# HongwenZhang/DaNet-DensePose2SMPL

Measured on AMD Instinct MI355X. Metric: images/sec fwd+bwd HRNet-W48+SMPL+IUV 256x256 bs32/GPU, higher is better.
Workload: dtype bf16; 1 GPU; full DaNet train step (HRNet-W48 + global and part-wise IUV heads + regressor nets + SMPL LBS (2 forward + 1 backward; the 2 label-side forwards belong to the untimed batch prologue) + IUV render + losses, fwd+bwd+Adam), 256x256, 32 img/GPU; convs bf16 MFMA fp32-acc, LBS/raster/losses fp32; global_batch=32, parallelism=dp1

## Files before the change

danet-densepose2smpl_amd/_lib.py:

```python
import ctypes
import os

_HERE = os.path.dirname(os.path.abspath(__file__))
LIB_PATH = os.environ.get('DANET_LIB') or os.path.join(_HERE, 'csrc', 'libdanet_hip.so')
_lib = None

c_f = ctypes.c_void_p
c_i = ctypes.c_int
c_sz = ctypes.c_size_t
c_fl = ctypes.c_float

_SIGNATURES = {
    'danet_version': (c_i, []),
    'danet_last_error': (ctypes.c_char_p, []),
    'danet_smpl_lbs_debug': (c_i, [c_f]),
    'danet_smpl_lbs_ctx_floats': (c_sz, [c_i]),
    'danet_smpl_lbs_fwd_ws_floats': (c_sz, [c_i, c_i, c_i]),
    'danet_smpl_lbs_bwd_ws_floats': (c_sz, [c_i, c_i, c_i]),
    'danet_smpl_lbs_ticket_words': (c_sz, [c_i]),
    'danet_smpl_lbs_forward': (c_i, [c_f, c_f, c_i] + [c_f] * 9 + [c_i] * 4 + [c_f] * 5 + [c_sz, c_f, c_f]),
    'danet_smpl_lbs_backward': (c_i, [c_f, c_f, c_i] + [c_f] * 7 + [c_i] * 4 + [c_f] * 7 + [c_sz, c_f, c_i, c_f]),
    'danet_smpl_lbs_backward_fused_ok': (c_i, [c_i, c_i, c_i]),
    'danet_iuv_raster_ws_bytes': (c_sz, [c_i, c_i, c_i]),
    'danet_iuv_raster_forward': (c_i, [c_f, c_f, c_i, c_i, c_f, c_i, c_f, c_f, c_i, c_fl, c_fl, c_i, c_f, c_f, c_f, c_f, c_sz, c_f]),
# ... 18 lines not shown
    'danet_conv_stem_ok': (c_i, [c_i] * 13),
    'danet_conv_stem_forward': (c_i, [c_f, c_f, c_f] + [c_i] * 7 + [c_f, c_f]),
    'danet_conv_stem_dgrad_ok': (c_i, [c_i] * 13),
    'danet_conv_stem_dgrad': (c_i, [c_f, c_f, c_f] + [c_i] * 7 + [c_f] * 5),
    'danet_conv3x3a_ok': (c_i, [c_i] * 11),
    'danet_conv3x3a': (c_i, [c_f, c_f, c_f] + [c_i] * 4 + [c_f] * 5 + [c_i, c_f, c_f]),
    'danet_conv3x3_stream_table_bytes': (c_sz, []),
    'danet_conv3x3_stream_tables': (c_i, [c_f, c_sz]),
    'danet_conv_pack_weights_batched': (c_i, [c_f, c_i, ctypes.c_long, ctypes.c_long, c_f]),
    'danet_conv_pack_job_bricks': (ctypes.c_long, [c_i] * 7),
    'danet_conv_forward_multi_ok': (c_i, [c_f, c_i]),
    'danet_conv_forward_multi_kernel': (c_i, [c_f, c_i]),
    'danet_conv_forward_multi': (c_i, [c_f, c_i, c_f]),
    'danet_conv_forward_multi_epi_ok': (c_i, [c_f, c_i]),
    'danet_conv_forward_multi_epi_kernel': (c_i, [c_f, c_i]),
    'danet_conv_forward_multi_epi': (c_i, [c_f, c_i, c_f]),
    'danet_conv_stem_forward_epi': (c_i, [c_f, c_f, c_f, c_f] + [c_i] * 8 + [c_f]),
    'danet_conv3x3a_forward_epi': (c_i, [c_f] * 5 + [c_i] * 4 + [c_f]),
    'danet_conv_bn_forward_multi_ok': (c_i, [c_f, c_i, c_f, c_f]),
    'danet_conv_bn_forward_multi': (c_i, [c_f, c_i, c_f, c_fl, c_fl, c_f, c_f, c_f]),
    'danet_conv_forward_kernel': (c_i, [c_i] * 15),
    'danet_conv_forward': (c_i, [c_f] * 4 + [c_i] * 16 + [c_f] * 6 + [c_i, c_f]),
    'danet_conv_wgrad_rows_ok': (c_i, [c_i] * 13),
    'danet_conv_wgrad_rows_ws_floats': (c_sz, [c_i] * 8),
    'danet_conv_wgrad_rows': (c_i, [c_f] * 4 + [c_sz] + [c_i] * 12 + [c_fl, c_f]),
    'danet_conv_wgrad3x3_ok': (c_i, [c_i] * 10),
    'danet_conv_wgrad3x3_pair_ok': (c_i, [c_i] * 11),
    'danet_conv_wgrad3x3_ws_floats': (c_sz, [c_i] * 7),
    'danet_conv_wgrad_multi_ws_floats': (c_sz, [c_f, c_i]),
    'danet_conv_wgrad_multi_ws_zero_from': (c_sz, [c_f, c_i]),
    'danet_conv_wgrad_multi': (c_i, [c_f, c_i, c_f, c_sz, c_fl, c_f]),
    'danet_conv_wgrad3x3_multi_ws_floats': (c_sz, [c_f, c_i]),
    'danet_conv_wgrad3x3_multi': (c_i, [c_f, c_i, c_f, c_sz, c_fl, c_f]),
    'danet_conv_wgrad3x3_kernel_id': (c_i, [c_i] * 7),
    'danet_conv_wgrad3x3': (c_i, [c_f] * 4 + [c_sz] + [c_i] * 7 + [c_fl, c_i, c_f]),
    'danet_conv_wgrad_ws_floats': (c_sz, [c_i] * 4),
    'danet_conv_wgrad_ws_floats_for': (c_sz, [c_i] * 13),
    'danet_conv_wgrad': (c_i, [c_f] * 4 + [c_sz] + [c_i] * 13 + [c_fl, c_i, c_f]),
    'danet_bn_forward': (c_i, [c_f, c_f, c_f, ctypes.c_int64, c_i] + [c_f] * 6 + [c_i, c_fl, c_fl, c_i, c_i, c_f, c_f]),
    'danet_bn_ws_floats': (c_sz, [c_i]),
    'danet_knob': (ctypes.c_long, [c_i, ctypes.c_long]),
    'danet_bn_acc_bytes': (c_i, []),
    'danet_channel_sum': (c_i, [c_f, ctypes.c_int64, c_i, c_f, c_i, c_i, c_f]),
    'danet_bn_forward_multi': (c_i, [c_f, c_i, c_fl, c_fl, c_f]),
    'danet_bn_backward_multi': (c_i, [c_f, c_i, c_f]),
    'danet_bn_backward_onepass_ok': (c_i, [c_f, c_i, c_i]),
    'danet_bn_backward_onepass_bar_words': (c_i, []),
    'danet_bn_backward_onepass': (c_i, [c_f, c_i, c_f, c_i, c_f]),
    'danet_bn_backward': (c_i, [c_f, c_f, c_f, ctypes.c_int64, c_i, c_f, c_f, c_i, c_f, c_f, c_f, c_f, c_i, c_i, c_f, c_f, c_f]),
    'danet_sum_relu_forward': (c_i, [ctypes.POINTER(ctypes.c_void_p), ctypes.POINTER(c_i), c_i, c_i, c_i, c_i, c_i, c_i, c_f, c_f]),
    'danet_sum_relu_backward': (c_i, [c_f, c_f, c_i, c_i, c_i, c_i, c_i, c_i, c_f, c_f]),
    'danet_sum_relu_backward_all': (c_i, [c_f, c_f] + [c_i] * 5 + [c_f] * 5),
    'danet_sum_relu_forward_multi': (c_i, [c_f, c_i, c_f]),
    'danet_sum_relu_backward_all_multi': (c_i, [c_f, c_i, c_f]),
    'danet_maxpool3x3s2_forward': (c_i, [c_f, c_f, c_f, c_i, c_i, c_i, c_i, c_f]),
    'danet_maxpool3x3s2_backward': (c_i, [c_f, c_f, c_f, c_i, c_i, c_i, c_i, c_f]),
    'danet_stn_gather_forward': (c_i, [c_f, c_f] + [c_i] * 8 + [c_f, c_f]),
    'danet_stn_gather_backward': (c_i, [c_f, c_f] + [c_i] * 8 + [c_f, c_f]),
    'danet_part_clean_forward': (c_i, [c_f, c_f, c_i, c_i, c_i, c_i, c_f, c_f]),
    'danet_part_clean_backward': (c_i, [c_f, c_f, c_f, c_i, c_i, c_i, c_i, c_f, c_f]),
    'danet_part_loss_forward': (c_i, [c_f] * 5 + [c_i] * 5 + [c_f, c_f]),
    'danet_part_loss_backward': (c_i, [c_f] * 6 + [c_i] * 5 + [c_f, c_f]),
    'danet_part_backward_fused': (c_i, [c_f] * 8 + [c_i] * 5 + [c_f, c_f]),
    'danet_part_gt_forward': (c_i, [c_f] * 5 + [c_i] * 4 + [c_f, c_f, c_f]),
    'danet_part_gt_backward': (c_i, [c_f] * 5 + [c_i] * 4 + [c_f, c_f]),
    'danet_iuv_global_forward': (c_i, [c_f] * 4 + [c_i, c_i] + [c_f] * 3 + [c_i] * 4 + [c_f] * 5),
# ... 301 lines not shown
```

danet-densepose2smpl_amd/csrc/conv_wgrad3x3.hip:

```cpp
#include <cstdlib>
#include "common.h"
#include "conv_common.h"

namespace {

using namespace danet_conv;

constexpr int TH = 4, TW = 8;
constexpr int halo_h(int st) { return st * (TH - 1) + 3; }
constexpr int halo_w(int st) { return st * (TW - 1) + 3; }

struct Wg3P {
    const bf16_t* x; const bf16_t* dy; float* part;
    float* direct;
    int B, H, W, Cin, Cout, groups, Cin_g, Cout_g;
    int IH, IW;
    int tiles_h, tiles_w, msplit;
    long nchunks;
    long x_bytes, dy_bytes;
};

typedef __attribute__((ext_vector_type(2))) unsigned v2u;

__device__ inline v2u tr_read(unsigned lds_byte_addr) {
    v2u r;
    asm volatile("ds_read_b64_tr_b16 %0, %1" : "=v"(r) : "v"(lds_byte_addr) : "memory");
    return r;
}

template <int CT, int NI, int ST, int SM = 0>
__device__ __forceinline__ void wgrad3x3_body(const Wg3P& p, const int bx, const int by, const int bz)
{
    constexpr bool PAIR = SM != 0;
// ... 143 lines not shown
            if (pair >= NPAIR || cin >= p.Cin_g) continue;
#pragma unroll
            for (int ct = 0; ct < CT; ++ct)
#pragma unroll
                for (int r = 0; r < 4; ++r) {
                    const int cout = co0 + ct * 16 + lg * 4 + r;
                    if (cout < p.Cout_g) dw[((size_t)cout * p.Cin_g + cin) * 9 + tap] = acc[pi][ct][r];
                }
        }
        return;
    }
    float* dst = p.part + ((size_t)bx * p.groups + g) * gsz;
#pragma unroll
    for (int pi = 0; pi < MAXP; ++pi) {
        const int pair = wave + 4 * pi;
        const int tap = pair / NI, ni = pair - tap * NI;
        const int cin = ci0 + ni * 16 + li;
        if (pair >= NPAIR || cin >= p.Cin_g) continue;
        float* row = dst + ((tap * p.Cout_g + co0 + lg * 4) * p.Cin_g + cin);
#pragma unroll
        for (int ct = 0; ct < CT; ++ct)
#pragma unroll
            for (int r = 0; r < 4; ++r)
                if (co0 + ct * 16 + lg * 4 + r < p.Cout_g) row[(ct * 16 + r) * p.Cin_g] = acc[pi][ct][r];
    }
}

template <int CT, int NI, int ST>
__global__ __launch_bounds__(256) void conv_wgrad3x3_kernel(Wg3P p)
{
    wgrad3x3_body<CT, NI, ST>(p, blockIdx.x, blockIdx.y, blockIdx.z);
}

constexpr int NPM = 20;
struct Wg3Multi { Wg3P p[NPM]; int start[NPM + 1]; int nyb[NPM]; int n; int xcd; };

template <int CT, int NI, int ST, int SM = 0>
__global__ __launch_bounds__(256) void conv_wgrad3x3_multi_kernel(Wg3Multi mp)
{
    int vb = (int)blockIdx.x;
    if (mp.xcd) {
        const int G = (int)gridDim.x, q = G >> 3, r = G & 7;
        const int x = vb & 7, slot = vb >> 3;
        vb = x * q + (x < r ? x : r) + slot;
    }
    int i = 0;
    while (i + 1 < mp.n && vb >= mp.start[i + 1]) ++i;
    const int l = vb - mp.start[i];
    const Wg3P& p = mp.p[i];
    const int bx = l % p.msplit, rest = l / p.msplit;
    wgrad3x3_body<CT, NI, ST, SM>(p, bx, rest % mp.nyb[i], rest / mp.nyb[i]);
}

struct Red3Multi { const float* part[NPM]; float* dw[NPM]; int G[NPM], Cout_g[NPM], Cin_g[NPM], msplit[NPM]; long start[NPM + 1]; int n; float beta; };

__global__ __launch_bounds__(256) void wgrad3x3_reduce_multi_kernel(Red3Multi rp)
{
    const long gidx = (long)blockIdx.x * 256 + threadIdx.x;
    if (gidx >= rp.start[rp.n]) return;
    int i = 0;
    while (i + 1 < rp.n && gidx >= rp.start[i + 1]) ++i;
    const long idx = gidx - rp.start[i], total = rp.start[i + 1] - rp.start[i];
    const float* part = rp.part[i];
    float s = 0.f;
    int sp = 0;
    for (; sp + 4 <= rp.msplit[i]; sp += 4) {
        const float v0 = part[(size_t)sp * total + idx], v1 = part[(size_t)(sp + 1) * total + idx];
        const float v2 = part[(size_t)(sp + 2) * total + idx], v3 = part[(size_t)(sp + 3) * total + idx];
        s += (v0 + v1) + (v2 + v3);
    }
    for (; sp < rp.msplit[i]; ++sp) s += part[(size_t)sp * total + idx];
    const int Cin_g = rp.Cin_g[i], Cout_g = rp.Cout_g[i];
    const int cin = (int)(idx % Cin_g);
    long rest = idx / Cin_g;
    const int cout = (int)(rest % Cout_g); rest /= Cout_g;
    const int tap = (int)(rest % 9), g = (int)(rest / 9);
    const size_t o = (((size_t)(g * Cout_g + cout)) * Cin_g + cin) * 9 + tap;
    float* dw = rp.dw[i];
    dw[o] = rp.beta != 0.f ? dw[o] * rp.beta + s : s;
}

__global__ __launch_bounds__(256) void wgrad3x3_reduce_kernel(const float* __restrict__ part, float* __restrict__ dw,
                                                               int G, int Cout_g, int Cin_g, int msplit, float beta)
{
    const long total = (long)G * Cout_g * Cin_g * 9;
    const long idx = (long)blockIdx.x * 256 + threadIdx.x;
    if (idx >= total) return;
    float s = 0.f;
    int sp = 0;
    for (; sp + 4 <= msplit; sp += 4) {
        const float v0 = part[(size_t)sp * total + idx], v1 = part[(size_t)(sp + 1) * total + idx];
        const float v2 = part[(size_t)(sp + 2) * total + idx], v3 = part[(size_t)(sp + 3) * total + idx];
        s += (v0 + v1) + (v2 + v3);
    }
    for (; sp < msplit; ++sp) s += part[(size_t)sp * total + idx];
    const int cin = (int)(idx % Cin_g);
    long rest = idx / Cin_g;
    const int cout = (int)(rest % Cout_g); rest /= Cout_g;
    const int tap = (int)(rest % 9), g = (int)(rest / 9);
    const size_t o = (((size_t)(g * Cout_g + cout)) * Cin_g + cin) * 9 + tap;
    dw[o] = beta != 0.f ? dw[o] * beta + s : s;
}

template <int CT, int NI, int ST>
int launch3(const Wg3P& p, hipStream_t st) {
    const int nco = (p.Cout_g + CT * 16 - 1) / (CT * 16), nci = (p.Cin_g + NI * 16 - 1) / (NI * 16);
    const size_t lds = 2 * (size_t)(TH * TW * CT * 32 + halo_h(ST) * halo_w(ST) * NI * 32);
    hipLaunchKernelGGL((conv_wgrad3x3_kernel<CT, NI, ST>), dim3(p.msplit, nco * nci, p.groups), dim3(256), lds, st, p);
    return 0;
}

inline int tiles3(int c) { return c <= 16 ? 1 : (c <= 32 ? 2 : ((c % 48 == 0 || c <= 48) ? 3 : 4)); }
// ... 60 lines not shown
    DANET_CHECK_ARG(danet_conv_wgrad3x3_ok(H, W, Cin, Cout, 3, 3, stride, 1, 1, groups), "conv_wgrad3x3: unsupported shape");
    Wg3P p;
    p.x = (const bf16_t*)x; p.dy = (const bf16_t*)dy; p.part = ws; p.direct = nullptr;
    p.IH = H; p.IW = W; H /= stride; W /= stride;
    p.B = B; p.H = H; p.W = W; p.Cin = Cin; p.Cout = Cout; p.groups = groups;
    p.Cin_g = Cin / groups; p.Cout_g = Cout / groups;
    p.tiles_h = H / TH; p.tiles_w = W / TW;
    p.nchunks = (long)B * p.tiles_h * p.tiles_w;
    p.x_bytes = (long)B * p.IH * p.IW * Cin * 2; p.dy_bytes = (long)B * H * W * Cout * 2;
    DANET_CHECK_ARG(p.x_bytes < (1L << 31) && p.dy_bytes < (1L << 31), "conv_wgrad3x3: tensors of 2 GB or more are not supported");
    int ct, ni;
    plan3(B, H, W, Cin, Cout, groups, &ct, &ni, &p.msplit);
    if (ws_floats < (size_t)p.msplit * Cout * p.Cin_g * 9)
        return danet::fail(DANET_ERR_WORKSPACE, "conv_wgrad3x3: workspace too small");
    hipStream_t st = (hipStream_t)stream;
    if (phase != 2) {
#define W3(a, b) if (ct == a && ni == b) { if (stride == 1) launch3<a, b, 1>(p, st); else launch3<a, b, 2>(p, st); } else
        W3(1, 1) W3(1, 2) W3(1, 3) W3(2, 1) W3(2, 2) W3(2, 3) W3(3, 1) W3(3, 2) W3(3, 3)
        return danet::fail(DANET_ERR_ARG, "conv_wgrad3x3: no kernel for tiles %dx%d", ct, ni);
#undef W3
        DANET_CHECK_LAUNCH("conv_wgrad3x3_kernel");
    }
    if (phase == 1) return DANET_OK;
    const long total = (long)Cout * p.Cin_g * 9;
    hipLaunchKernelGGL(wgrad3x3_reduce_kernel, dim3(danet::cdiv(total, 256)), dim3(256), 0, st, ws, dw, groups, p.Cout_g,
                       p.Cin_g, p.msplit, beta);
    DANET_CHECK_LAUNCH("wgrad3x3_reduce_kernel");
    return DANET_OK;
}


struct Wg3Job { const void* x; const void* dy; float* dw; int B, H, W, Cin, Cout, groups, stride; };

static long multi_target_blocks() {
    if (const char* e = getenv("DANET_WGRAD3_MULTI_BLOCKS")) return atol(e);
    return 768;
}

static inline double wg3_weight(int Cout, int Cin_g) { const double p = (double)Cout * Cin_g; return p < 2304.0 ? 2304.0 : p; }
static void plan_multi(const Wg3Job* jobs, const int* idx, int cnt, int ct, int ni, int* msplit) {
    auto chunks_of = [](const Wg3Job& j) -> long {
        const int sm = wg3_small(j.B, j.H, j.W, j.stride);
        return sm ? (long)(j.B / (sm == 4 ? 2 : 8)) : (long)j.B * (j.H / j.stride / TH) * (j.W / j.stride / TW);
    };
    double tot = 0;
    for (int k = 0; k < cnt; ++k) {
        const Wg3Job& j = jobs[idx[k]];
        tot += (double)chunks_of(j) * wg3_weight(j.Cout, j.Cin / j.groups);
    }
    const long target = multi_target_blocks();
    for (int k = 0; k < cnt; ++k) {
        const Wg3Job& j = jobs[idx[k]];
        const int Cout_g = j.Cout / j.groups, Cin_g = j.Cin / j.groups;
        const long other = (long)((Cout_g + ct * 16 - 1) / (ct * 16)) * ((Cin_g + ni * 16 - 1) / (ni * 16)) * j.groups;
        const long nchunks = chunks_of(j);
        const double w = (double)nchunks * wg3_weight(j.Cout, Cin_g);
        long ms = (long)(target * (w / tot) / other + 0.5);
        if (ms > nchunks / 4) ms = nchunks / 4;
        if (ms < 1) ms = 1;
        msplit[k] = (int)ms;
    }
}

static int multi_foreach_launch(const Wg3Job* jobs, int n, float* ws, size_t ws_floats, float beta, hipStream_t st, size_t* need_out)
{
    size_t used = 0;
    bool done[4096];
    if (n > 4096) return danet::fail(DANET_ERR_ARG, "conv_wgrad3x3_multi: too many jobs (%d)", n);
    for (int i = 0; i < n; ++i) done[i] = false;
    for (int i = 0; i < n; ++i) {
        if (done[i]) continue;
        int ct, ni, dummy;
        const int stride = jobs[i].stride;
        const int sm = wg3_small(jobs[i].B, jobs[i].H, jobs[i].W, stride);
        const bool pair = sm != 0;
        plan3(jobs[i].B, jobs[i].H / stride, jobs[i].W / stride, jobs[i].Cin, jobs[i].Cout, jobs[i].groups, &ct, &ni, &dummy);
        static const int npm_env = getenv("DANET_WGRAD3_NPM") ? atoi(getenv("DANET_WGRAD3_NPM")) : 0;
        const int npm = npm_env > 0 && npm_env < NPM ? npm_env : NPM;
        int idx[NPM], cnt = 0;
        for (int k = i; k < n && cnt < npm; ++k) {
            if (done[k] || jobs[k].stride != stride || wg3_small(jobs[k].B, jobs[k].H, jobs[k].W, stride) != sm) continue;
            int c2, n2;
            plan3(jobs[k].B, jobs[k].H / stride, jobs[k].W / stride, jobs[k].Cin, jobs[k].Cout, jobs[k].groups, &c2, &n2, &dummy);
            if (c2 == ct && n2 == ni) { idx[cnt++] = k; done[k] = true; }
        }
        int msplit[NPM];
        plan_multi(jobs, idx, cnt, ct, ni, msplit);
        Wg3Multi mp; Red3Multi rp;
        static const bool xcd_order = getenv("DANET_WGRAD3_XCD") && atoi(getenv("DANET_WGRAD3_XCD")) != 0;
        mp.n = cnt; rp.n = cnt; rp.beta = beta; mp.xcd = xcd_order ? 1 : 0;
        mp.start[0] = 0; rp.start[0] = 0;
        for (int k = 0; k < cnt; ++k) {
            const Wg3Job& j = jobs[idx[k]];
            Wg3P& p = mp.p[k];
            static const bool no_direct = getenv("DANET_WGRAD3_NO_DIRECT") != nullptr;
            const bool direct = msplit[k] == 1 && beta == 0.f && !no_direct;
            p.x = (const bf16_t*)j.x; p.dy = (const bf16_t*)j.dy; p.part = (ws && !direct) ? ws + used : nullptr;
            p.direct = direct ? j.dw : nullptr;
            p.IH = j.H; p.IW = j.W;
            p.B = j.B; p.H = j.H / stride; p.W = j.W / stride; p.Cin = j.Cin; p.Cout = j.Cout; p.groups = j.groups;
            if (pair) { p.B = j.B / (sm == 4 ? 2 : 8); p.H = 4; p.W = 8; p.IH = 4 * stride; p.IW = 8 * stride; }
            p.Cin_g = j.Cin / j.groups; p.Cout_g = j.Cout / j.groups;
            p.tiles_h = p.H / TH; p.tiles_w = p.W / TW;
            p.nchunks = (long)p.B * p.tiles_h * p.tiles_w;
            p.x_bytes = (long)j.B * j.H * j.W * j.Cin * 2; p.dy_bytes = (long)j.B * (j.H / stride) * (j.W / stride) * j.Cout * 2;
            p.msplit = msplit[k];
            const int nyb = ((p.Cout_g + ct * 16 - 1) / (ct * 16)) * ((p.Cin_g + ni * 16 - 1) / (ni * 16));
            mp.nyb[k] = nyb;
            mp.start[k + 1] = mp.start[k] + msplit[k] * nyb * j.groups;
            const long total = (long)j.Cout * p.Cin_g * 9;
            rp.part[k] = p.part; rp.dw[k] = j.dw; rp.G[k] = j.groups; rp.Cout_g[k] = p.Cout_g; rp.Cin_g[k] = p.Cin_g; rp.msplit[k] = msplit[k];
            rp.start[k + 1] = rp.start[k] + (direct ? 0 : total);
            if (!direct || !ws) used += (size_t)msplit[k] * total;
            if (ws && !(p.x_bytes < (1L << 31) && p.dy_bytes < (1L << 31)))
                return danet::fail(DANET_ERR_ARG, "conv_wgrad3x3_multi: tensors of 2 GB or more are not supported");
        }
        if (!ws) continue;
        if (used > ws_floats) return danet::fail(DANET_ERR_WORKSPACE, "conv_wgrad3x3_multi: workspace too small");
        const int phw = stride * ((sm ? sm : 4) - 1) + 3;
        const size_t lds = 2 * (size_t)(TH * TW * ct * 32 + (sm ? (TH / sm) * phw * (TW / sm) * phw : halo_h(stride) * halo_w(stride)) * ni * 32);
        const dim3 grid((unsigned)mp.start[cnt]);
        if (pair) {
#define W3P(a, b) if (ct == a && ni == b) { \
            if (stride == 1 && sm == 4) hipLaunchKernelGGL((conv_wgrad3x3_multi_kernel<a, b, 1, 4>), grid, dim3(256), lds, st, mp); \
            else if (stride == 2 && sm == 4) hipLaunchKernelGGL((conv_wgrad3x3_multi_kernel<a, b, 2, 4>), grid, dim3(256), lds, st, mp); \
            else if (stride == 1) hipLaunchKernelGGL((conv_wgrad3x3_multi_kernel<a, b, 1, 2>), grid, dim3(256), lds, st, mp); \
            else hipLaunchKernelGGL((conv_wgrad3x3_multi_kernel<a, b, 2, 2>), grid, dim3(256), lds, st, mp); } else
            W3P(2, 2) W3P(2, 3) W3P(3, 2) W3P(3, 3) W3P(1, 1) W3P(1, 2) W3P(2, 1) W3P(1, 3) W3P(3, 1)
            return danet::fail(DANET_ERR_ARG, "conv_wgrad3x3_multi: no pair-mode kernel for tiles %dx%d", ct, ni);
#undef W3P
        } else
#define W3M(a, b) if (ct == a && ni == b) { \
            if (stride == 1) hipLaunchKernelGGL((conv_wgrad3x3_multi_kernel<a, b, 1>), grid, dim3(256), lds, st, mp); \
            else hipLaunchKernelGGL((conv_wgrad3x3_multi_kernel<a, b, 2>), grid, dim3(256), lds, st, mp); } else
        W3M(1, 1) W3M(1, 2) W3M(1, 3) W3M(2, 1) W3M(2, 2) W3M(2, 3) W3M(3, 1) W3M(3, 2) W3M(3, 3)
        return danet::fail(DANET_ERR_ARG, "conv_wgrad3x3_multi: no kernel for tiles %dx%d", ct, ni);
#undef W3M
        DANET_CHECK_LAUNCH("conv_wgrad3x3_multi_kernel");
        if (rp.start[cnt] > 0) {
            hipLaunchKernelGGL(wgrad3x3_reduce_multi_kernel, dim3((unsigned)danet::cdiv(rp.start[cnt], 256)), dim3(256), 0, st, rp);
            DANET_CHECK_LAUNCH("wgrad3x3_reduce_multi_kernel");
        }
    }
    if (need_out) *need_out = used;
    return DANET_OK;
}

extern "C" size_t danet_conv_wgrad3x3_multi_ws_floats(const void* jobs, int n)
{
    size_t need = 0;
    if (!jobs || n <= 0) return 0;
    multi_foreach_launch((const Wg3Job*)jobs, n, nullptr, 0, 0.f, nullptr, &need);
    return need;
}

extern "C" int danet_conv_wgrad3x3_multi(const void* jobs, int n, float* ws, size_t ws_floats, float beta, void* stream)
{
    DANET_ENTER();
    DANET_CHECK_ARG(jobs && n > 0 && ws, "conv_wgrad3x3_multi: bad arguments");
    const Wg3Job* jb = (const Wg3Job*)jobs;
    for (int i = 0; i < n; ++i)
        DANET_CHECK_ARG(jb[i].x && jb[i].dy && jb[i].dw && jb[i].B > 0 &&
                        (danet_conv_wgrad3x3_ok(jb[i].H, jb[i].W, jb[i].Cin, jb[i].Cout, 3, 3, jb[i].stride, 1, 1, jb[i].groups) ||
                         danet_conv_wgrad3x3_pair_ok(jb[i].B, jb[i].H, jb[i].W, jb[i].Cin, jb[i].Cout, 3, 3, jb[i].stride, 1, 1, jb[i].groups)),
                        "conv_wgrad3x3_multi: job %d is not a supported 3x3 problem", i);
    return multi_foreach_launch(jb, n, ws, ws_floats, beta, (hipStream_t)stream, nullptr);
}
```

include/danet_hip.h:

```cpp
#ifndef DANET_HIP_H
#define DANET_HIP_H

#include <stddef.h>
#include <stdint.h>

#ifdef __cplusplus
extern "C" {
#endif

#define DANET_OK 0
#define DANET_ERR_ARG (-1)
#define DANET_ERR_HIP (-2)
#define DANET_ERR_WORKSPACE (-3)

int danet_version(void);
const char* danet_last_error(void);

size_t danet_smpl_lbs_ctx_floats(int B);
size_t danet_smpl_lbs_fwd_ws_floats(int B, int V, int NE);
size_t danet_smpl_lbs_bwd_ws_floats(int B, int V, int NB);
size_t danet_smpl_lbs_ticket_words(int B);

int danet_smpl_lbs_forward(const float* betas, const float* rotmats, int B,
                           const float* v_template, const float* shapedirs, const float* posedirs,
// ... 171 lines not shown
       DANET_KNOB_BN_BLOCK_BYTES = 15, DANET_KNOB_C3S_BALANCE = 16, DANET_KNOB_C3S_TILE_COST = 17,
       DANET_KNOB_G3 = 18  };
long danet_knob(int id, long value);
int danet_conv3x3_stream_plan(int B, int H, int W, int Cin, int Cout, int nprob);
size_t danet_conv3x3_stream_table_bytes(void);
int danet_conv3x3_stream_tables(void* workspace, size_t bytes);
int danet_conv_stem_ok(int B, int H, int W, int Cin, int OH, int OW, int Cout, int R, int S, int stride, int pad, int dil, int groups);
int danet_conv_stem_forward(const void* x, const void* wp, void* y, int B, int H, int W, int Cin, int OH, int OW, int Cout,
                            float* bn_sums, void* stream);
int danet_conv_stem_forward_epi(const void* x, const void* wp, const float* bias, void* y, int B, int H, int W, int Cin, int OH, int OW,
                                int Cout, int relu, void* stream);
int danet_conv_stem_dgrad_ok(int B, int H, int W, int Cin, int OH, int OW, int Cout, int R, int S, int stride, int pad, int dil, int groups);
int danet_conv_stem_dgrad(const void* dy, const void* wp, void* dx, int B, int H, int W, int Cin, int OH, int OW, int Cout,
                          const void* bn_x, const void* bn_y, const float* bn_saved, float* bn_red, void* stream);
int danet_conv3x3a_ok(int B, int H, int W, int Cin, int Cout, int R, int S, int stride, int pad, int dil, int groups);
int danet_conv3x3a(const void* x, const void* wp, void* y, int B, int H, int W, int transposed, float* bn_sums,
                   const void* bn_x, const void* bn_y, const float* bn_saved, float* bn_red, int bn_gate, const void* addend, void* stream);
int danet_conv3x3a_forward_epi(const void* x, const void* wp, const float* bias, const void* addend, void* y, int B, int H, int W,
                               int relu, void* stream);
void danet_conv3x3_debug(int* dev_buf);
int danet_conv_forward_multi(const void* jobs, int n, void* stream);
int danet_conv_forward_kernel(int B, int H, int W, int Cin, int OH, int OW, int Cout, int R, int S,
                              int stride, int pad, int dil, int groups, int transposed, int out_fp32);
int danet_conv_forward(const void* x, const void* wp, const float* bias, void* y,
                       int B, int H, int W, int Cin, int OH, int OW, int Cout,
                       int R, int S, int stride, int pad, int dil, int groups, int transposed,
                       int relu, int out_fp32, float* bn_sums,
                       const void* bn_x, const void* bn_y, const float* bn_saved, float* bn_red, const void* addend,
                       int bn_gate, void* stream);
int danet_conv_wgrad3x3_ok(int H, int W, int Cin, int Cout, int R, int S, int stride, int pad, int dil, int groups);
int danet_conv_wgrad3x3_pair_ok(int B, int H, int W, int Cin, int Cout, int R, int S, int stride, int pad, int dil, int groups);
size_t danet_conv_wgrad3x3_ws_floats(int B, int H, int W, int Cin, int Cout, int groups, int stride);
size_t danet_conv_wgrad3x3_multi_ws_floats(const void* jobs, int n);
size_t danet_conv_wgrad_multi_ws_floats(const void* jobs, int n);
size_t danet_conv_wgrad_multi_ws_zero_from(const void* jobs, int n);
int danet_conv_wgrad_multi(const void* jobs, int n, float* ws, size_t ws_floats, float beta, void* stream);
int danet_conv_wgrad3x3_multi(const void* jobs, int n, float* ws, size_t ws_floats, float beta, void* stream);
int danet_conv_wgrad3x3_kernel_id(int B, int H, int W, int Cin, int Cout, int groups, int stride);
int danet_conv_wgrad3x3(const void* x, const void* dy, float* dw, float* ws, size_t ws_floats,
                        int B, int H, int W, int Cin, int Cout, int groups, int stride, float beta, int phase , void* stream);
int danet_conv_wgrad_rows_ok(int B, int H, int W, int Cin, int OH, int OW, int Cout, int R, int S, int stride, int pad, int dil, int groups);
size_t danet_conv_wgrad_rows_ws_floats(int B, int OH, int OW, int Cin, int Cout, int R, int S, int groups);
int danet_conv_wgrad_rows(const void* x, const void* dy, float* dw, float* ws, size_t ws_floats,
                          int B, int H, int W, int Cin, int OH, int OW, int Cout,
                          int R, int S, int stride, int pad, int groups, float beta, void* stream);
size_t danet_conv_wgrad_ws_floats(int Cout, int Cin_g, int R, int S);
size_t danet_conv_wgrad_ws_floats_for(int B, int H, int W, int Cin, int OH, int OW, int Cout, int R, int S, int stride, int pad, int dil, int groups);
int danet_conv_wgrad(const void* x, const void* dy, float* dw, float* ws, size_t ws_floats,
                     int B, int H, int W, int Cin, int OH, int OW, int Cout,
                     int R, int S, int stride, int pad, int dil, int groups, float beta, int ws_is_zero, void* stream);

int danet_bn_forward(const void* x, const void* res, void* y, int64_t M, int C,
                     const float* gamma, const float* beta, float* running_mean, float* running_var,
                     float* saved, float* sums_ws, int ws_is_zero, float momentum, float eps, int training, int relu,
                     void* relu_mask, void* stream);
size_t danet_bn_ws_floats(int C);
int danet_bn_acc_bytes(void);
int danet_bn_backward(const void* dy, const void* x, const void* y, int64_t M, int C,
                      const float* gamma, const float* saved, int relu,
                      void* dx, void* dres, float* dparam, float* red_ws, int ws_is_zero,
                      int mask_mode, const void* relu_mask, const float* beta, void* stream);
int danet_bn_forward_multi(const void* jobs, int n, float momentum, float eps, void* stream);
int danet_bn_backward_multi(const void* jobs, int n, void* stream);
int danet_bn_backward_onepass_bar_words(void);
int danet_bn_backward_onepass_ok(const void* jobs, int n, int max_blocks);
int danet_bn_backward_onepass(const void* jobs, int n, void* bar, int max_blocks, void* stream);
// ... 179 lines not shown
```

Before: 1334 images/sec.

## Batch 3x3 wgrad multi-launch via device-side job tables and larger grouped launches

Replaces the by-value kernel-argument job arrays, capped at 20 jobs, with a device-resident entry table and a per-block map. The table is uploaded by small copy kernels, so up to 60 jobs share one launch, and jobs are sorted longest-first within each launch. The reduce kernel becomes float4-vectorised with per-job block ranges and deeper unrolling over splits. This cuts launch count and per-block linear job search, but adds table-upload kernels and more workspace, and relies on 16-byte alignment.

```diff
diff --git a/danet-densepose2smpl_amd/_lib.py b/danet-densepose2smpl_amd/_lib.py
--- a/danet-densepose2smpl_amd/_lib.py
+++ b/danet-densepose2smpl_amd/_lib.py
@@ -74,6 +74,7 @@
     'danet_conv_wgrad_multi': (c_i, [c_f, c_i, c_f, c_sz, c_fl, c_f]),
     'danet_conv_wgrad3x3_multi_ws_floats': (c_sz, [c_f, c_i]),
     'danet_conv_wgrad3x3_multi': (c_i, [c_f, c_i, c_f, c_sz, c_fl, c_f]),
+    'danet_conv_wgrad3x3_multi_plan': (c_i, [c_f, c_i, c_f, c_i]),
     'danet_conv_wgrad3x3_kernel_id': (c_i, [c_i] * 7),
     'danet_conv_wgrad3x3': (c_i, [c_f] * 4 + [c_sz] + [c_i] * 7 + [c_fl, c_i, c_f]),
     'danet_conv_wgrad_ws_floats': (c_sz, [c_i] * 4),
diff --git a/danet-densepose2smpl_amd/csrc/conv_wgrad3x3.hip b/danet-densepose2smpl_amd/csrc/conv_wgrad3x3.hip
--- a/danet-densepose2smpl_amd/csrc/conv_wgrad3x3.hip
+++ b/danet-densepose2smpl_amd/csrc/conv_wgrad3x3.hip
@@ -1,4 +1,8 @@
+#include <algorithm>
+#include <cstdint>
 #include <cstdlib>
+#include <cstring>
+#include <vector>
 #include "common.h"
 #include "conv_common.h"
 
@@ -208,52 +212,77 @@
     wgrad3x3_body<CT, NI, ST>(p, blockIdx.x, blockIdx.y, blockIdx.z);
 }
 
-constexpr int NPM = 20;
-struct Wg3Multi { Wg3P p[NPM]; int start[NPM + 1]; int nyb[NPM]; int n; int xcd; };
+struct Wg3Ent {
+    Wg3P p;
+    float* dw;
+    int nyb, wg0;
+    int rblk0, rblks;
+};
+static_assert(sizeof(Wg3Ent) % 8 == 0, "table entries are copied as 8-byte words");
+
+__device__ __forceinline__ int wg3_map_at(const unsigned* __restrict__ map, int b) {
+    return (int)((map[b >> 1] >> ((b & 1) * 16)) & 0xffffu);
+}
 
 template <int CT, int NI, int ST, int SM = 0>
-__global__ __launch_bounds__(256) void conv_wgrad3x3_multi_kernel(Wg3Multi mp)
-{
-    int vb = (int)blockIdx.x;
-    if (mp.xcd) {
-        const int G = (int)gridDim.x, q = G >> 3, r = G & 7;
-        const int x = vb & 7, slot = vb >> 3;
-        vb = x * q + (x < r ? x : r) + slot;
-    }
-    int i = 0;
-    while (i + 1 < mp.n && vb >= mp.start[i + 1]) ++i;
-    const int l = vb - mp.start[i];
-    const Wg3P& p = mp.p[i];
+__global__ __launch_bounds__(256) void conv_wgrad3x3_multi_kernel(const Wg3Ent* __restrict__ ent, const unsigned* __restrict__ wgmap)
+{
+    const int vb = (int)blockIdx.x;
+    const Wg3Ent* const e = ent + wg3_map_at(wgmap, vb);
+    const Wg3P p = e->p;
+    const int l = vb - e->wg0, nyb = e->nyb;
     const int bx = l % p.msplit, rest = l / p.msplit;
-    wgrad3x3_body<CT, NI, ST, SM>(p, bx, rest % mp.nyb[i], rest / mp.nyb[i]);
-}
-
-struct Red3Multi { const float* part[NPM]; float* dw[NPM]; int G[NPM], Cout_g[NPM], Cin_g[NPM], msplit[NPM]; long start[NPM + 1]; int n; float beta; };
-
-__global__ __launch_bounds__(256) void wgrad3x3_reduce_multi_kernel(Red3Multi rp)
-{
-    const long gidx = (long)blockIdx.x * 256 + threadIdx.x;
-    if (gidx >= rp.start[rp.n]) return;
-    int i = 0;
-    while (i + 1 < rp.n && gidx >= rp.start[i + 1]) ++i;
-    const long idx = gidx - rp.start[i], total = rp.start[i + 1] - rp.start[i];
-    const float* part = rp.part[i];
-    float s = 0.f;
-    int sp = 0;
-    for (; sp + 4 <= rp.msplit[i]; sp += 4) {
-        const float v0 = part[(size_t)sp * total + idx], v1 = part[(size_t)(sp + 1) * total + idx];
-        const float v2 = part[(size_t)(sp + 2) * total + idx], v3 = part[(size_t)(sp + 3) * total + idx];
-        s += (v0 + v1) + (v2 + v3);
-    }
-    for (; sp < rp.msplit[i]; ++sp) s += part[(size_t)sp * total + idx];
-    const int Cin_g = rp.Cin_g[i], Cout_g = rp.Cout_g[i];
-    const int cin = (int)(idx % Cin_g);
-    long rest = idx / Cin_g;
-    const int cout = (int)(rest % Cout_g); rest /= Cout_g;
-    const int tap = (int)(rest % 9), g = (int)(rest / 9);
-    const size_t o = (((size_t)(g * Cout_g + cout)) * Cin_g + cin) * 9 + tap;
-    float* dw = rp.dw[i];
-    dw[o] = rp.beta != 0.f ? dw[o] * rp.beta + s : s;
+    wgrad3x3_body<CT, NI, ST, SM>(p, bx, rest % nyb, rest / nyb);
+}
+
+constexpr int WG3_PIECE = 224;
+struct Wg3Piece { uint4 v[WG3_PIECE]; };
+
+__global__ __launch_bounds__(256) void wgrad3x3_table_kernel(uint4* __restrict__ dst, const Wg3Piece pc, const int n16)
+{
+    const int t = threadIdx.x;
+    if (t < n16) dst[t] = pc.v[t];
+}
+
+__device__ __forceinline__ float4 add4(const float4 a, const float4 b) { return make_float4(a.x + b.x, a.y + b.y, a.z + b.z, a.w + b.w); }
+
+__global__ __launch_bounds__(256) void wgrad3x3_reduce_multi_kernel(const Wg3Ent* __restrict__ ent, const unsigned* __restrict__ rmap,
+                                                                     const float beta)
+{
+    const int vb = (int)blockIdx.x, t = threadIdx.x;
+    const Wg3Ent* const e = ent + wg3_map_at(rmap, vb);
+    const int msplit = e->p.msplit, Cin_g = e->p.Cin_g, Cout_g = e->p.Cout_g;
+    const long total = (long)e->p.groups * 9 * Cout_g * Cin_g;
+    const float* const part = e->p.part;
+    float* const dw = e->dw;
+    const long step = (long)e->rblks * 1024;
+    for (long idx = (long)(vb - e->rblk0) * 1024 + t * 4; idx < total; idx += step) {
+        float4 s = make_float4(0.f, 0.f, 0.f, 0.f);
+        int sp = 0;
+        for (; sp + 16 <= msplit; sp += 16) {
+            float4 v[16];
+#pragma unroll
+            for (int k = 0; k < 16; ++k) v[k] = *reinterpret_cast<const float4*>(part + (size_t)(sp + k) * total + idx);
+#pragma unroll
+            for (int k = 0; k < 16; k += 4) s = add4(s, add4(add4(v[k], v[k + 1]), add4(v[k + 2], v[k + 3])));
+        }
+        for (; sp + 4 <= msplit; sp += 4) {
+            const float4 v0 = *reinterpret_cast<const float4*>(part + (size_t)sp * total + idx);
+            const float4 v1 = *reinterpret_cast<const float4*>(part + (size_t)(sp + 1) * total + idx);
+            const float4 v2 = *reinterpret_cast<const float4*>(part + (size_t)(sp + 2) * total + idx);
+            const float4 v3 = *reinterpret_cast<const float4*>(part + (size_t)(sp + 3) * total + idx);
+            s = add4(s, add4(add4(v0, v1), add4(v2, v3)));
+        }
+        for (; sp < msplit; ++sp) s = add4(s, *reinterpret_cast<const float4*>(part + (size_t)sp * total + idx));
+        const int cin = (int)(idx % Cin_g);
+        long rest = idx / Cin_g;
+        const int cout = (int)(rest % Cout_g); rest /= Cout_g;
+        const int tap = (int)(rest % 9), g = (int)(rest / 9);
+        float* const o = dw + (((size_t)(g * Cout_g + cout)) * Cin_g + cin) * 9 + tap;
+        const float v[4] = {s.x, s.y, s.z, s.w};
+#pragma unroll
+        for (int k = 0; k < 4; ++k) o[k * 9] = beta != 0.f ? o[k * 9] * beta + v[k] : v[k];
+    }
 }
 
 __global__ __launch_bounds__(256) void wgrad3x3_reduce_kernel(const float* __restrict__ part, float* __restrict__ dw,
@@ -380,29 +409,37 @@
 
 struct Wg3Job { const void* x; const void* dy; float* dw; int B, H, W, Cin, Cout, groups, stride; };
 
+constexpr int PLAN_UNIT = 20;
+#ifndef DANET_WG3_LAUNCH_UNITS
+#define DANET_WG3_LAUNCH_UNITS 3
+#endif
+constexpr int LAUNCH_UNITS = DANET_WG3_LAUNCH_UNITS;
 static long multi_target_blocks() {
     if (const char* e = getenv("DANET_WGRAD3_MULTI_BLOCKS")) return atol(e);
     return 768;
 }
 
 static inline double wg3_weight(int Cout, int Cin_g) { const double p = (double)Cout * Cin_g; return p < 2304.0 ? 2304.0 : p; }
+static inline long wg3_chunks(const Wg3Job& j) {
+    const int sm = wg3_small(j.B, j.H, j.W, j.stride);
+    return sm ? (long)(j.B / (sm == 4 ? 2 : 8)) : (long)j.B * (j.H / j.stride / TH) * (j.W / j.stride / TW);
+}
+static inline long wg3_other(const Wg3Job& j, int ct, int ni) {
+    const int Cout_g = j.Cout / j.groups, Cin_g = j.Cin / j.groups;
+    return (long)((Cout_g + ct * 16 - 1) / (ct * 16)) * ((Cin_g + ni * 16 - 1) / (ni * 16)) * j.groups;
+}
 static void plan_multi(const Wg3Job* jobs, const int* idx, int cnt, int ct, int ni, int* msplit) {
-    auto chunks_of = [](const Wg3Job& j) -> long {
-        const int sm = wg3_small(j.B, j.H, j.W, j.stride);
-        return sm ? (long)(j.B / (sm == 4 ? 2 : 8)) : (long)j.B * (j.H / j.stride / TH) * (j.W / j.stride / TW);
-    };
     double tot = 0;
     for (int k = 0; k < cnt; ++k) {
         const Wg3Job& j = jobs[idx[k]];
-        tot += (double)chunks_of(j) * wg3_weight(j.Cout, j.Cin / j.groups);
+        tot += (double)wg3_chunks(j) * wg3_weight(j.Cout, j.Cin / j.groups);
     }
     const long target = multi_target_blocks();
     for (int k = 0; k < cnt; ++k) {
         const Wg3Job& j = jobs[idx[k]];
-        const int Cout_g = j.Cout / j.groups, Cin_g = j.Cin / j.groups;
-        const long other = (long)((Cout_g + ct * 16 - 1) / (ct * 16)) * ((Cin_g + ni * 16 - 1) / (ni * 16)) * j.groups;
-        const long nchunks = chunks_of(j);
-        const double w = (double)nchunks * wg3_weight(j.Cout, Cin_g);
+        const long other = wg3_other(j, ct, ni);
+        const long nchunks = wg3_chunks(j);
+        const double w = (double)nchunks * wg3_weight(j.Cout, j.Cin / j.groups);
         long ms = (long)(target * (w / tot) / other + 0.5);
         if (ms > nchunks / 4) ms = nchunks / 4;
         if (ms < 1) ms = 1;
@@ -410,96 +447,216 @@
     }
 }
 
-static int multi_foreach_launch(const Wg3Job* jobs, int n, float* ws, size_t ws_floats, float beta, hipStream_t st, size_t* need_out)
-{
-    size_t used = 0;
+struct Wg3Launch { int first, cnt, ct, ni, stride, sm; };
+struct Wg3Plan {
+    std::vector<int> order, msplit;
+    std::vector<Wg3Launch> launches;
+};
+
+static int build_plan(const Wg3Job* jobs, int n, Wg3Plan& pl)
+{
     bool done[4096];
     if (n > 4096) return danet::fail(DANET_ERR_ARG, "conv_wgrad3x3_multi: too many jobs (%d)", n);
     for (int i = 0; i < n; ++i) done[i] = false;
+    pl.order.reserve(n); pl.msplit.reserve(n);
+    std::vector<int> grp, ms;
     for (int i = 0; i < n; ++i) {
         if (done[i]) continue;
         int ct, ni, dummy;
         const int stride = jobs[i].stride;
         const int sm = wg3_small(jobs[i].B, jobs[i].H, jobs[i].W, stride);
-        const bool pair = sm != 0;
         plan3(jobs[i].B, jobs[i].H / stride, jobs[i].W / stride, jobs[i].Cin, jobs[i].Cout, jobs[i].groups, &ct, &ni, &dummy);
-        static const int npm_env = getenv("DANET_WGRAD3_NPM") ? atoi(getenv("DANET_WGRAD3_NPM")) : 0;
-        const int npm = npm_env > 0 && npm_env < NPM ? npm_env : NPM;
-        int idx[NPM], cnt = 0;
-        for (int k = i; k < n && cnt < npm; ++k) {
+        grp.clear();
+        for (int k = i; k < n; ++k) {
             if (done[k] || jobs[k].stride != stride || wg3_small(jobs[k].B, jobs[k].H, jobs[k].W, stride) != sm) continue;
             int c2, n2;
             plan3(jobs[k].B, jobs[k].H / stride, jobs[k].W / stride, jobs[k].Cin, jobs[k].Cout, jobs[k].groups, &c2, &n2, &dummy);
-            if (c2 == ct && n2 == ni) { idx[cnt++] = k; done[k] = true; }
-        }
-        int msplit[NPM];
-        plan_multi(jobs, idx, cnt, ct, ni, msplit);
-        Wg3Multi mp; Red3Multi rp;
-        static const bool xcd_order = getenv("DANET_WGRAD3_XCD") && atoi(getenv("DANET_WGRAD3_XCD")) != 0;
-        mp.n = cnt; rp.n = cnt; rp.beta = beta; mp.xcd = xcd_order ? 1 : 0;
-        mp.start[0] = 0; rp.start[0] = 0;
-        for (int k = 0; k < cnt; ++k) {
-            const Wg3Job& j = jobs[idx[k]];
-            Wg3P& p = mp.p[k];
-            static const bool no_direct = getenv("DANET_WGRAD3_NO_DIRECT") != nullptr;
-            const bool direct = msplit[k] == 1 && beta == 0.f && !no_direct;
-            p.x = (const bf16_t*)j.x; p.dy = (const bf16_t*)j.dy; p.part = (ws && !direct) ? ws + used : nullptr;
+            if (c2 == ct && n2 == ni) { grp.push_back(k); done[k] = true; }
+        }
+        const int all = (int)grp.size();
+        ms.assign(all, 1);
+        for (int off = 0; off < all; off += PLAN_UNIT)
+            plan_multi(jobs, grp.data() + off, std::min(PLAN_UNIT, all - off), ct, ni, ms.data() + off);
+        const int per = LAUNCH_UNITS > 0 ? LAUNCH_UNITS * PLAN_UNIT : all;
+        for (int off = 0; off < all; off += per) {
+            const int cnt = std::min(per, all - off);
+            std::vector<int> pos(cnt);
+            for (int k = 0; k < cnt; ++k) pos[k] = off + k;
+            auto len = [&](int k) { const long c = wg3_chunks(jobs[grp[k]]); return (c + ms[k] - 1) / ms[k]; };
+            std::stable_sort(pos.begin(), pos.end(), [&](int a, int b) { return len(a) > len(b); });
+            pl.launches.push_back(Wg3Launch{(int)pl.order.size(), cnt, ct, ni, stride, sm});
+            for (int k = 0; k < cnt; ++k) { pl.order.push_back(grp[pos[k]]); pl.msplit.push_back(ms[pos[k]]); }
+        }
+    }
+    return DANET_OK;
+}
+
+static inline int wg3_red_blocks(long total, int nred) {
+    return (int)std::min((long)danet::cdiv(total, 1024), (long)std::max(16, 4096 / std::max(1, nred)));
+}
+static inline size_t wg3_table_bytes(int cnt, long wgs) {
+    const size_t rb = (size_t)std::max(16L * cnt, 4096L);
+    return (((size_t)cnt * sizeof(Wg3Ent) + 15) & ~(size_t)15) + ((2 * (size_t)wgs + 15) & ~(size_t)15) + ((2 * rb + 15) & ~(size_t)15);
+}
+
+static void plan_sizes(const Wg3Job* jobs, const Wg3Plan& pl, size_t* part_floats, size_t* table_floats)
+{
+    size_t part = 0, tab = 0;
+    for (const Wg3Launch& L : pl.launches) {
+        long wgs = 0;
+        for (int k = L.first; k < L.first + L.cnt; ++k) {
+            const Wg3Job& j = jobs[pl.order[k]];
+            part += (size_t)pl.msplit[k] * j.Cout * (j.Cin / j.groups) * 9;
+            wgs += pl.msplit[k] * wg3_other(j, L.ct, L.ni);
+        }
+        tab += wg3_table_bytes(L.cnt, wgs);
+    }
+    *part_floats = (part + 3) & ~(size_t)3;
+    *table_floats = tab / 4;
+}
+
+template <int CT, int NI>
+static void launch_multi(int stride, int sm, dim3 grid, size_t lds, hipStream_t st, const Wg3Ent* ent, const unsigned* wgmap)
+{
+    if (sm == 4 && stride == 1) hipLaunchKernelGGL((conv_wgrad3x3_multi_kernel<CT, NI, 1, 4>), grid, dim3(256), lds, st, ent, wgmap);
+    else if (sm == 4) hipLaunchKernelGGL((conv_wgrad3x3_multi_kernel<CT, NI, 2, 4>), grid, dim3(256), lds, st, ent, wgmap);
+    else if (sm == 2 && stride == 1) hipLaunchKernelGGL((conv_wgrad3x3_multi_kernel<CT, NI, 1, 2>), grid, dim3(256), lds, st, ent, wgmap);
+    else if (sm == 2) hipLaunchKernelGGL((conv_wgrad3x3_multi_kernel<CT, NI, 2, 2>), grid, dim3(256), lds, st, ent, wgmap);
+    else if (stride == 1) hipLaunchKernelGGL((conv_wgrad3x3_multi_kernel<CT, NI, 1>), grid, dim3(256), lds, st, ent, wgmap);
+    else hipLaunchKernelGGL((conv_wgrad3x3_multi_kernel<CT, NI, 2>), grid, dim3(256), lds, st, ent, wgmap);
+}
+
+static int multi_launch(const Wg3Job* jobs, int n, float* ws, size_t ws_floats, float beta, hipStream_t st)
+{
+    Wg3Plan pl;
+    if (int rc = build_plan(jobs, n, pl)) return rc;
+    size_t part_floats, table_floats;
+    plan_sizes(jobs, pl, &part_floats, &table_floats);
+    if (ws_floats < part_floats + table_floats) return danet::fail(DANET_ERR_WORKSPACE, "conv_wgrad3x3_multi: workspace too small");
+    for (int i = 0; i < n; ++i)
+        if (!((long)jobs[i].B * jobs[i].H * jobs[i].W * jobs[i].Cin * 2 < (1L << 31) &&
+              (long)jobs[i].B * (jobs[i].H / jobs[i].stride) * (jobs[i].W / jobs[i].stride) * jobs[i].Cout * 2 < (1L << 31)))
+            return danet::fail(DANET_ERR_ARG, "conv_wgrad3x3_multi: tensors of 2 GB or more are not supported");
+
+    static const bool no_direct = getenv("DANET_WGRAD3_NO_DIRECT") != nullptr;
+    unsigned char* const tab_dev = reinterpret_cast<unsigned char*>(ws + part_floats);
+    struct Offs { size_t ent, wgmap, rmap; long wgs, rblks; };
+    std::vector<Offs> offs(pl.launches.size());
+    std::vector<unsigned char> blob;
+    size_t used = 0;
+    for (size_t li = 0; li < pl.launches.size(); ++li) {
+        const Wg3Launch& L = pl.launches[li];
+        const int stride = L.stride, sm = L.sm;
+        std::vector<Wg3Ent> ent(L.cnt);
+        int nred = 0;
+        for (int k = 0; k < L.cnt; ++k) nred += !(pl.msplit[L.first + k] == 1 && beta == 0.f && !no_direct);
+        long wgs = 0, rblks = 0;
+        for (int k = 0; k < L.cnt; ++k) {
+            const Wg3Job& j = jobs[pl.order[L.first + k]];
+            const int msplit = pl.msplit[L.first + k];
+            Wg3Ent& e = ent[k];
+            Wg3P& p = e.p;
+            const bool direct = msplit == 1 && beta == 0.f && !no_direct;
+            const long total = (long)j.Cout * (j.Cin / j.groups) * 9;
+            p.x = (const bf16_t*)j.x; p.dy = (const bf16_t*)j.dy; p.part = direct ? nullptr : ws + used;
             p.direct = direct ? j.dw : nullptr;
             p.IH = j.H; p.IW = j.W;
             p.B = j.B; p.H = j.H / stride; p.W = j.W / stride; p.Cin = j.Cin; p.Cout = j.Cout; p.groups = j.groups;
-            if (pair) { p.B = j.B / (sm == 4 ? 2 : 8); p.H = 4; p.W = 8; p.IH = 4 * stride; p.IW = 8 * stride; }
+            if (sm) { p.B = j.B / (sm == 4 ? 2 : 8); p.H = 4; p.W = 8; p.IH = 4 * stride; p.IW = 8 * stride; }
             p.Cin_g = j.Cin / j.groups; p.Cout_g = j.Cout / j.groups;
             p.tiles_h = p.H / TH; p.tiles_w = p.W / TW;
             p.nchunks = (long)p.B * p.tiles_h * p.tiles_w;
             p.x_bytes = (long)j.B * j.H * j.W * j.Cin * 2; p.dy_bytes = (long)j.B * (j.H / stride) * (j.W / stride) * j.Cout * 2;
-            p.msplit = msplit[k];
-            const int nyb = ((p.Cout_g + ct * 16 - 1) / (ct * 16)) * ((p.Cin_g + ni * 16 - 1) / (ni * 16));
-            mp.nyb[k] = nyb;
-            mp.start[k + 1] = mp.start[k] + msplit[k] * nyb * j.groups;
-            const long total = (long)j.Cout * p.Cin_g * 9;
-            rp.part[k] = p.part; rp.dw[k] = j.dw; rp.G[k] = j.groups; rp.Cout_g[k] = p.Cout_g; rp.Cin_g[k] = p.Cin_g; rp.msplit[k] = msplit[k];
-            rp.start[k + 1] = rp.start[k] + (direct ? 0 : total);
-            if (!direct || !ws) used += (size_t)msplit[k] * total;
-            if (ws && !(p.x_bytes < (1L << 31) && p.dy_bytes < (1L << 31)))
-                return danet::fail(DANET_ERR_ARG, "conv_wgrad3x3_multi: tensors of 2 GB or more are not supported");
-        }
-        if (!ws) continue;
-        if (used > ws_floats) return danet::fail(DANET_ERR_WORKSPACE, "conv_wgrad3x3_multi: workspace too small");
+            p.msplit = msplit;
+            e.dw = j.dw;
+            e.nyb = (int)(wg3_other(j, L.ct, L.ni) / j.groups);
+            e.wg0 = (int)wgs;
+            e.rblk0 = (int)rblks;
+            e.rblks = direct ? 0 : wg3_red_blocks(total, nred);
+            wgs += (long)msplit * e.nyb * j.groups;
+            rblks += e.rblks;
+            if (!direct) used += (size_t)msplit * total;
+        }
+        if (wgs >= (1L << 31)) return danet::fail(DANET_ERR_ARG, "conv_wgrad3x3_multi: too many workgroups");
+        Offs& o = offs[li];
+        o.wgs = wgs; o.rblks = rblks;
+        o.ent = blob.size();
+        blob.resize(o.ent + (((size_t)L.cnt * sizeof(Wg3Ent) + 15) & ~(size_t)15), 0);
+        memcpy(blob.data() + o.ent, ent.data(), (size_t)L.cnt * sizeof(Wg3Ent));
+        o.wgmap = blob.size();
+        blob.resize(o.wgmap + ((2 * (size_t)wgs + 15) & ~(size_t)15), 0);
+        o.rmap = blob.size();
+        blob.resize(o.rmap + ((2 * (size_t)rblks + 15) & ~(size_t)15), 0);
+        unsigned short* const wm = reinterpret_cast<unsigned short*>(blob.data() + o.wgmap);
+        unsigned short* const rm = reinterpret_cast<unsigned short*>(blob.data() + o.rmap);
+        for (int k = 0; k < L.cnt; ++k) {
+            const long w1 = k + 1 < L.cnt ? ent[k + 1].wg0 : wgs;
+            for (long b = ent[k].wg0; b < w1; ++b) wm[b] = (unsigned short)k;
+            for (int b = 0; b < ent[k].rblks; ++b) rm[ent[k].rblk0 + b] = (unsigned short)k;
+        }
+    }
+    if (used > part_floats || blob.size() > table_floats * 4)
+        return danet::fail(DANET_ERR_WORKSPACE, "conv_wgrad3x3_multi: plan and sizing disagree (%zu / %zu floats, %zu / %zu table bytes)",
+                           used, part_floats, blob.size(), table_floats * 4);
+    if ((reinterpret_cast<uintptr_t>(ws) & 15) != 0) return danet::fail(DANET_ERR_ARG, "conv_wgrad3x3_multi: ws must be 16-byte aligned");
+
+    for (size_t at = 0; at < blob.size(); at += sizeof(Wg3Piece)) {
+        Wg3Piece pc{};
+        const size_t nb = std::min(sizeof(Wg3Piece), blob.size() - at);
+        memcpy(&pc, blob.data() + at, nb);
+        hipLaunchKernelGGL(wgrad3x3_table_kernel, dim3(1), dim3(256), 0, st, reinterpret_cast<uint4*>(tab_dev + at), pc, (int)(nb / 16));
+        DANET_CHECK_LAUNCH("wgrad3x3_table_kernel");
+    }
+    for (size_t li = 0; li < pl.launches.size(); ++li) {
+        const Wg3Launch& L = pl.launches[li];
+        const Offs& o = offs[li];
+        const int ct = L.ct, ni = L.ni, stride = L.stride, sm = L.sm;
+        const Wg3Ent* const ent = reinterpret_cast<const Wg3Ent*>(tab_dev + o.ent);
         const int phw = stride * ((sm ? sm : 4) - 1) + 3;
         const size_t lds = 2 * (size_t)(TH * TW * ct * 32 + (sm ? (TH / sm) * phw * (TW / sm) * phw : halo_h(stride) * halo_w(stride)) * ni * 32);
-        const dim3 grid((unsigned)mp.start[cnt]);
-        if (pair) {
-#define W3P(a, b) if (ct == a && ni == b) { \
-            if (stride == 1 && sm == 4) hipLaunchKernelGGL((conv_wgrad3x3_multi_kernel<a, b, 1, 4>), grid, dim3(256), lds, st, mp); \
-            else if (stride == 2 && sm == 4) hipLaunchKernelGGL((conv_wgrad3x3_multi_kernel<a, b, 2, 4>), grid, dim3(256), lds, st, mp); \
-            else if (stride == 1) hipLaunchKernelGGL((conv_wgrad3x3_multi_kernel<a, b, 1, 2>), grid, dim3(256), lds, st, mp); \
-            else hipLaunchKernelGGL((conv_wgrad3x3_multi_kernel<a, b, 2, 2>), grid, dim3(256), lds, st, mp); } else
-            W3P(2, 2) W3P(2, 3) W3P(3, 2) W3P(3, 3) W3P(1, 1) W3P(1, 2) W3P(2, 1) W3P(1, 3) W3P(3, 1)
-            return danet::fail(DANET_ERR_ARG, "conv_wgrad3x3_multi: no pair-mode kernel for tiles %dx%d", ct, ni);
-#undef W3P
-        } else
-#define W3M(a, b) if (ct == a && ni == b) { \
-            if (stride == 1) hipLaunchKernelGGL((conv_wgrad3x3_multi_kernel<a, b, 1>), grid, dim3(256), lds, st, mp); \
-            else hipLaunchKernelGGL((conv_wgrad3x3_multi_kernel<a, b, 2>), grid, dim3(256), lds, st, mp); } else
+        const dim3 grid((unsigned)o.wgs);
+#define W3M(a, b) if (ct == a && ni == b) launch_multi<a, b>(stride, sm, grid, lds, st, ent, reinterpret_cast<const unsigned*>(tab_dev + o.wgmap)); else
         W3M(1, 1) W3M(1, 2) W3M(1, 3) W3M(2, 1) W3M(2, 2) W3M(2, 3) W3M(3, 1) W3M(3, 2) W3M(3, 3)
         return danet::fail(DANET_ERR_ARG, "conv_wgrad3x3_multi: no kernel for tiles %dx%d", ct, ni);
 #undef W3M
         DANET_CHECK_LAUNCH("conv_wgrad3x3_multi_kernel");
-        if (rp.start[cnt] > 0) {
-            hipLaunchKernelGGL(wgrad3x3_reduce_multi_kernel, dim3((unsigned)danet::cdiv(rp.start[cnt], 256)), dim3(256), 0, st, rp);
+        if (o.rblks > 0) {
+            hipLaunchKernelGGL(wgrad3x3_reduce_multi_kernel, dim3((unsigned)o.rblks), dim3(256), 0, st, ent,
+                               reinterpret_cast<const unsigned*>(tab_dev + o.rmap), beta);
             DANET_CHECK_LAUNCH("wgrad3x3_reduce_multi_kernel");
         }
     }
-    if (need_out) *need_out = used;
     return DANET_OK;
 }
 
 extern "C" size_t danet_conv_wgrad3x3_multi_ws_floats(const void* jobs, int n)
 {
-    size_t need = 0;
     if (!jobs || n <= 0) return 0;
-    multi_foreach_launch((const Wg3Job*)jobs, n, nullptr, 0, 0.f, nullptr, &need);
-    return need;
+    Wg3Plan pl;
+    if (build_plan((const Wg3Job*)jobs, n, pl)) return 0;
+    size_t part_floats, table_floats;
+    plan_sizes((const Wg3Job*)jobs, pl, &part_floats, &table_floats);
+    return part_floats + table_floats;
+}
+
+extern "C" int danet_conv_wgrad3x3_multi_plan(const void* jobs, int n, int* out, int cap)
+{
+    if (!jobs || n <= 0 || !out || cap < n) return -1;
+    const Wg3Job* jb = (const Wg3Job*)jobs;
+    for (int i = 0; i < n; ++i)
+        if (!(jb[i].B > 0 && (danet_conv_wgrad3x3_ok(jb[i].H, jb[i].W, jb[i].Cin, jb[i].Cout, 3, 3, jb[i].stride, 1, 1, jb[i].groups) ||
+                              danet_conv_wgrad3x3_pair_ok(jb[i].B, jb[i].H, jb[i].W, jb[i].Cin, jb[i].Cout, 3, 3, jb[i].stride, 1, 1, jb[i].groups))))
+            return -1;
+    Wg3Plan pl;
+    if (build_plan(jb, n, pl)) return -1;
+    for (size_t li = 0; li < pl.launches.size(); ++li) {
+        const Wg3Launch& L = pl.launches[li];
+        for (int k = L.first; k < L.first + L.cnt; ++k) {
+            int* o = out + 4 * (size_t)pl.order[k];
+            o[0] = (int)li; o[1] = pl.msplit[k]; o[2] = (int)(pl.msplit[k] * wg3_other(jb[pl.order[k]], L.ct, L.ni)); o[3] = pl.msplit[k] == 1;
+        }
+    }
+    return (int)pl.launches.size();
 }
 
 extern "C" int danet_conv_wgrad3x3_multi(const void* jobs, int n, float* ws, size_t ws_floats, float beta, void* stream)
@@ -512,5 +669,5 @@
                         (danet_conv_wgrad3x3_ok(jb[i].H, jb[i].W, jb[i].Cin, jb[i].Cout, 3, 3, jb[i].stride, 1, 1, jb[i].groups) ||
                          danet_conv_wgrad3x3_pair_ok(jb[i].B, jb[i].H, jb[i].W, jb[i].Cin, jb[i].Cout, 3, 3, jb[i].stride, 1, 1, jb[i].groups)),
                         "conv_wgrad3x3_multi: job %d is not a supported 3x3 problem", i);
-    return multi_foreach_launch(jb, n, ws, ws_floats, beta, (hipStream_t)stream, nullptr);
-}
+    return multi_launch(jb, n, ws, ws_floats, beta, (hipStream_t)stream);
+}
diff --git a/include/danet_hip.h b/include/danet_hip.h
--- a/include/danet_hip.h
+++ b/include/danet_hip.h
@@ -227,6 +227,7 @@
 int danet_conv_wgrad3x3_pair_ok(int B, int H, int W, int Cin, int Cout, int R, int S, int stride, int pad, int dil, int groups);
 size_t danet_conv_wgrad3x3_ws_floats(int B, int H, int W, int Cin, int Cout, int groups, int stride);
 size_t danet_conv_wgrad3x3_multi_ws_floats(const void* jobs, int n);
+int danet_conv_wgrad3x3_multi_plan(const void* jobs, int n, int* out, int cap);
 size_t danet_conv_wgrad_multi_ws_floats(const void* jobs, int n);
 size_t danet_conv_wgrad_multi_ws_zero_from(const void* jobs, int n);
 int danet_conv_wgrad_multi(const void* jobs, int n, float* ws, size_t ws_floats, float beta, void* stream);
```

After: 1342 images/sec (median of 6 runs). About the same (+0.6%).
